# dhansmair/flamingo-mini

Measured on AMD Instinct MI355X. Metric: images/sec (fwd+bwd) flamingo-mini bs=32, higher is better.
Workload: dtype bf16

## Files before the change

flamingo-mini_amd/csrc/ff_api.hip:

```cpp
#include <stdarg.h>
#include <stdio.h>
#include <math.h>
#include <stdlib.h>
#include "ff_common.h"
#include "ff_internal.h"

namespace ff {

static thread_local char g_err[512] = "";
void set_error(const char* fmt, ...) {
    va_list ap;
    va_start(ap, fmt);
    vsnprintf(g_err, sizeof(g_err), fmt, ap);
    va_end(ap);
}
#ifdef FF_DEBUG
int dbg_switch(const char* name, int dflt) {
    const char* e = getenv(name);
    return e ? atoi(e) : dflt;
}
#endif
int check_launch(const char* what) {
    hipError_t e = hipGetLastError();
    if (e != hipSuccess) {
// ... 50 lines not shown
};
static void rs_take_layer_saved(const RsDims& s, Arena& a, RsLayerSaved& L) {
    const size_t rows_q = s.Mq, rows_kv = s.Mkv;
    L.mean_l = a.take<float>(rows_q * 4);
    L.rstd_l = a.take<float>(rows_q * 4);
    L.kv_in = a.take(rows_kv * s.D * s.es);
    L.Qs = a.take(rows_q * s.inner * s.es);
    L.K = a.take(rows_kv * s.inner * s.es);
    L.V = a.take(rows_kv * s.inner * s.es);
    L.lse = a.take<float>((size_t)s.Bn * s.H * s.q * 4);
    L.O = a.take(rows_q * s.inner * s.es);
    L.x_mid = a.take(rows_q * s.D * s.es);
    L.mean_f = a.take<float>(rows_q * 4);
    L.rstd_f = a.take<float>(rows_q * 4);
    L.xn_f = a.take(rows_q * s.D * s.es);
    L.Hpre = a.take(rows_q * s.ffi * s.es);
    L.Aact = a.take(rows_q * s.ffi * s.es);
}
static size_t rs_saved_layout(const RsDims& s, void* base, size_t cap, RsSaved& o) {
    Arena a(base, cap);
    const size_t rows_q = s.Mq;
    o.mean_m = a.take<float>((size_t)s.Mf * 4);
    o.rstd_m = a.take<float>((size_t)s.Mf * 4);
    for (int l = 0; l < s.depth; l++) {
        o.L[l].x_in = l == 0 ? nullptr : a.take(rows_q * s.D * s.es);
        rs_take_layer_saved(s, a, o.L[l]);
    }
    o.x_last = a.take(rows_q * s.D * s.es);
    o.mean_o = a.take<float>(rows_q * 4);
    o.rstd_o = a.take<float>(rows_q * 4);
    return align_up(a.used);
}

static size_t rs_ws_bytes(const RsDims& s) {
    size_t w = 0;
    auto g = [&](int M, int N, int K, int nz) { w = std::max(w, gemm_workspace_bytes(s.dt, M, N, K, nz, 0)); };
    g(s.Mq, s.inner, s.D, 1); g(s.Mkv, s.inner, s.D, 2); g(s.Mq, s.D, s.inner, 1); g(s.Mq, s.ffi, s.D, 1); g(s.Mq, s.D, s.ffi, 1);
    for (int nz = 1; nz <= 4; nz++) {
        g(s.D, s.ffi, s.Mq, nz); g(s.ffi, s.D, s.Mq, nz); g(s.D, s.inner, s.Mq, nz); g(s.inner, s.D, s.Mq, nz); g(s.inner, s.D, s.Mkv, nz);
    }
    g(s.Mkv, s.D, s.inner, 1);
    w = std::max(w, layernorm_bwd_workspace(s.Mf, s.D));
    w = std::max(w, layernorm_bwd_workspace(s.Mq, s.D));
    w = std::max(w, rows_reduce_workspace(s.Mq, s.D, s.q, 1));
    w = std::max(w, rows_reduce_workspace(s.Mf, s.D, s.F, s.v));
    return align_up(w) + align_up(s.attn_ws);
}
struct RsChain {
    void *ws, *dxn, *dO, *dkv, *dln;
    size_t ws_bytes, gws;
    float* attn_ws;
};
struct RsLayerGrads {
    void *dx_mid, *dH, *dQs, *dK, *dV;
};
static void rs_take_ws(const RsDims& s, Arena& a, RsChain& c) {
    c.ws_bytes = rs_ws_bytes(s);
    c.ws = a.take(c.ws_bytes);
    c.gws = c.ws_bytes - align_up(s.attn_ws);
    c.attn_ws = c.ws ? (float*)((char*)c.ws + c.gws) : nullptr;
}
static void rs_take_chain(const RsDims& s, Arena& a, RsChain& c) {
    c.dxn = a.take((size_t)s.Mq * s.D * s.es);
    c.dO = a.take((size_t)s.Mq * s.inner * s.es);
    c.dkv = a.take((size_t)s.Mkv * s.D * s.es);
    c.dln = a.take((size_t)s.Mq * s.D * s.es);
}
static void rs_take_layer_grads(const RsDims& s, Arena& a, RsLayerGrads& g) {
    g.dx_mid = a.take((size_t)s.Mq * s.D * s.es);
    g.dH = a.take((size_t)s.Mq * s.ffi * s.es);
    g.dQs = a.take((size_t)s.Mq * s.inner * s.es);
    g.dK = a.take((size_t)s.Mkv * s.inner * s.es);
    g.dV = a.take((size_t)s.Mkv * s.inner * s.es);
}
static void rs_take_ln_partials(const RsDims& s, Arena& a, bool deferrable, float** lnp) {
    for (int i = 0; i < 3; i++) lnp[i] = deferrable ? a.take<float>(layernorm_bwd_partial_bytes(i == 2 ? s.Mf : s.Mq, s.D)) : nullptr;
}

struct RsScratch {
    RsChain c;
    void *dx0, *dxf;
    void* dx_out[kMaxDepth];
    RsLayerGrads L[kMaxDepth];
    float* lnp[3 * kMaxDepth + 1];
};
static size_t rs_scratch_layout(const RsDims& s, void* base, size_t cap, bool bwd, RsScratch& o) {
    Arena a(base, cap);
    rs_take_ws(s, a, o.c);
    if (bwd) {
        o.dx0 = a.take((size_t)s.Mq * s.D * s.es);
        rs_take_chain(s, a, o.c);
        o.dxf = a.take((size_t)s.Mf * s.D * s.es);
        for (int l = 0; l < s.depth; l++) {
            o.dx_out[l] = a.take((size_t)s.Mq * s.D * s.es);
            rs_take_layer_grads(s, a, o.L[l]);
        }
        static const int defer_ln = dbg_switch("FF_DEFER_LN", 1);
        const bool lnd = defer_ln != 0 && layernorm_bwd_deferrable(s.dt, s.D);
        for (int l = 0; l < s.depth; l++) rs_take_ln_partials(s, a, lnd, o.lnp + 3 * l);
        o.lnp[3 * s.depth] = lnd ? a.take<float>(layernorm_bwd_partial_bytes(s.Mq, s.D)) : nullptr;
    }
    return align_up(a.used);
}

static int rs_check(const ff_resampler_desc* d) {
    FF_CHECK(d, FF_ERR_SHAPE, "resampler: null descriptor");
    FF_CHECK(d->dtype == FF_DTYPE_F32 || d->dtype == FF_DTYPE_BF16, FF_ERR_UNSUPPORTED, "resampler: dtype %d", d->dtype);
    FF_CHECK(d->batch > 0 && d->n_frames > 0 && d->n_tokens > 0 && d->dim > 0 && d->depth > 0 && d->depth <= kMaxDepth && d->heads > 0 &&
                 d->dim_head > 0 && d->num_latents > 0 && d->ff_mult > 0,
             FF_ERR_SHAPE, "resampler: bad dimensions");
    FF_CHECK(d->n_frames <= d->num_time_embeds, FF_ERR_SHAPE, "resampler: %d frames > num_time_embeds %d (perceiver_resampler.py:166)",
             d->n_frames, d->num_time_embeds);
    FF_CHECK(d->act >= FF_ACT_GELU && d->act <= FF_ACT_RELU, FF_ERR_SHAPE, "resampler: act %d", d->act);
    return FF_OK;
}

static ff_attn_desc rs_attn_desc(const RsDims& s) {
    ff_attn_desc a = {};
    a.dtype = s.dt; a.batch = s.Bn; a.heads = s.H; a.dim_head = s.dh; a.n_q = s.q; a.n_kv = s.R; a.mode = FF_ATTN_DENSE;
    const ff_strides sq = {(long long)s.q * s.inner, s.inner, s.dh}, sk = {(long long)s.R * s.inner, s.inner, s.dh};
    a.q = sq; a.o = sq; a.dq = sq; a.dout = sq;
    a.k = sk; a.v = sk; a.dk = sk; a.dv = sk;
    return a;
}

static int rs_media_stats(const RsDims& s, const void* x_f, const void* tpe, float* mean_m, float* rstd_m, hipStream_t st) {
    return layernorm_fwd(s.ln_media(s.pD), x_f, tpe, nullptr, nullptr, nullptr, mean_m, rstd_m, st);
}

static int rs_layer_forward(const RsDims& s, const void* const* p, const void* x_f, const void* tpe, float* mean_m, float* rstd_m, const void* x_in,
                            RowMap x_map, void* x_out, const RsLayerSaved& L, void* ws, size_t ws_bytes, hipStream_t st) {
    const RowMap pD = s.pD, pI = s.pI, pF = s.pF;
    void* kv_lat_base = s.kv_latent_rows(L.kv_in);
    {
        LnArgs a = s.ln_media(s.kv_media);
        a.stats_given = 1;
        FF_TRY(layernorm_fwd(a, x_f, tpe, p[0], p[1], L.kv_in, mean_m, rstd_m, st));
    }
    FF_TRY(layernorm_fwd(ln_args(s.dt, s.Mq, s.D, x_map, s.kv_lat, pD), x_in, nullptr, p[2], p[3], kv_lat_base, L.mean_l, L.rstd_l, st));
    FF_TRY(Gemm(s.dt, s.Mq, s.inner, s.D).a(0, s.kv_lat).b(0, pD).c(pI).scale(s.scale).problem(kv_lat_base, p[4], L.Qs).run(ws, ws_bytes, st));
    FF_TRY(Gemm(s.dt, s.Mkv, s.inner, s.D).a(0, pD).b(0, pD).c(pI).problem(L.kv_in, p[5], L.K).problem(L.kv_in, p[6], L.V).run(ws, ws_bytes, st));
    FF_TRY(attention_fwd(rs_attn_desc(s), L.Qs, L.K, L.V, nullptr, L.O, L.lse, st));
    FF_TRY(Gemm(s.dt, s.Mq, s.D, s.inner).a(0, pI).b(0, pI).c(pD).res_map(x_map).problem(L.O, p[7], L.x_mid, nullptr, nullptr, x_in).run(ws, ws_bytes, st));
    FF_TRY(layernorm_fwd(s.ln_latents(), L.x_mid, nullptr, p[8], p[9], L.xn_f, L.mean_f, L.rstd_f, st));
    FF_TRY(Gemm(s.dt, s.Mq, s.ffi, s.D).a(0, pD).b(0, pD).c(pF).act(s.act).problem(L.xn_f, p[10], L.Aact, L.Hpre).run(ws, ws_bytes, st));
    return Gemm(s.dt, s.Mq, s.D, s.ffi).a(0, pF).b(0, pF).c(pD).problem(L.Aact, p[11], x_out, nullptr, nullptr, L.x_mid).run(ws, ws_bytes, st);
}

static int rs_final_norm(const RsDims& s, const void* x_last, const void* gamma, const void* beta, void* out, float* mean, float* rstd, hipStream_t st) {
    return layernorm_fwd(s.ln_latents(), x_last, nullptr, gamma, beta, out, mean, rstd, st);
}

static int rs_ln_bwd(const RsChain& W, float* partial, LnPending* pending, const LnArgs& a, const void* dy, const void* x, const void* add,
                     const void* gamma, const float* mean, const float* rstd, void* dx, const void* dx_res, void* dg, void* db, hipStream_t st) {
    if (partial)
        return layernorm_bwd(a, dy, x, add, gamma, mean, rstd, dx, dx_res, dg, db, partial, layernorm_bwd_partial_bytes(a.rows, a.cols), st, nullptr, pending);
    return layernorm_bwd(a, dy, x, add, gamma, mean, rstd, dx, dx_res, dg, db, W.ws, W.gws, st);
}

static int rs_layer_backward(const RsDims& s, const void* const* p, void* const* g, const void* x_f, const void* tpe, const float* mean_m,
                             const float* rstd_m, const void* x_in, RowMap x_map, const RsLayerSaved& L, const void* dx_out, void* dx_in,
                             void* dx_f, const void* dx_f_res, const RsChain& W, const RsLayerGrads& T, float* const* lnp, LnPending* ln_sets,
                             hipStream_t st) {
    const RowMap pD = s.pD, pI = s.pI, pF = s.pF;
    FF_TRY(Gemm(s.dt, s.Mq, s.ffi, s.D).a(0, pD).b(1, pF).c(pF).act_bwd(s.act).problem(dx_out, p[11], T.dH, nullptr, L.Hpre).run(W.ws, W.gws, st));
    FF_TRY(Gemm(s.dt, s.Mq, s.D, s.ffi).a(0, pF).b(1, pD).c(pD).problem(T.dH, p[10], W.dxn).run(W.ws, W.gws, st));
    FF_TRY(rs_ln_bwd(W, lnp[0], &ln_sets[0], s.ln_latents(), W.dxn, L.x_mid, nullptr, p[8], L.mean_f, L.rstd_f, T.dx_mid, dx_out, g[8], g[9], st));
    FF_TRY(Gemm(s.dt, s.Mq, s.inner, s.D).a(0, pD).b(1, pI).c(pI).problem(T.dx_mid, p[7], W.dO).run(W.ws, W.gws, st));
    FF_TRY(attention_bwd(rs_attn_desc(s), L.Qs, L.K, L.V, nullptr, L.O, W.dO, L.lse, T.dQs, T.dK, T.dV, W.attn_ws, s.attn_ws, st));
    FF_TRY(Gemm(s.dt, s.Mkv, s.D, s.inner).a(0, pI).b(1, pD).c(pD).problem(T.dK, p[5], W.dkv).run(W.ws, W.gws, st));
    FF_TRY(Gemm(s.dt, s.Mkv, s.D, s.inner).a(0, pI).b(1, pD).c(pD).problem(T.dV, p[6], W.dkv, nullptr, nullptr, W.dkv).run(W.ws, W.gws, st));
    FF_TRY(Gemm(s.dt, s.Mq, s.D, s.inner).a(0, pI).b(1, pD).c(pD).res_map(s.kv_lat).scale(s.scale)
               .problem(T.dQs, p[4], W.dln, nullptr, nullptr, s.kv_latent_rows(W.dkv)).run(W.ws, W.gws, st));
    FF_TRY(rs_ln_bwd(W, lnp[1], &ln_sets[1], ln_args(s.dt, s.Mq, s.D, x_map, pD, pD), W.dln, x_in, nullptr, p[2], L.mean_l, L.rstd_l, dx_in, T.dx_mid, g[2],
                     g[3], st));
    return rs_ln_bwd(W, lnp[2], &ln_sets[2], s.ln_media(s.kv_media), W.dkv, x_f, tpe, p[0], mean_m, rstd_m, dx_f, dx_f_res, g[0], g[1], st);
}

static int rs_input_grads(const RsDims& s, const void* dx0, const void* dxf, void* d_latents, void* d_tpe, void* ws, size_t ws_bytes, hipStream_t st) {
    FF_TRY(rows_reduce(s.dt, s.Mq, s.D, s.pD, s.q, 1, dx0, d_latents, ws, ws_bytes, st));
    if (s.nte > s.T) FF_TRY(zero_bytes((char*)d_tpe + (size_t)s.T * s.D * s.es, (size_t)(s.nte - s.T) * s.D * s.es, st));
    return rows_reduce(s.dt, s.Mf, s.D, s.pD, s.F, s.v, dxf, d_tpe, ws, ws_bytes, st);
}

static int resampler_fwd(const ff_resampler_desc* d, const void* x_f, const void* const* P, void* out, void* saved, size_t saved_bytes,
                         void* scratch, size_t scratch_bytes, hipStream_t st) {
    FF_TRY(rs_check(d));
    FF_CHECK(x_f && P && out && saved && scratch, FF_ERR_SHAPE, "resampler_fwd: null argument");
    const RsDims s(*d);
    RsSaved S;
    RsScratch W;
    FF_CHECK(rs_saved_layout(s, saved, saved_bytes, S) <= saved_bytes, FF_ERR_WORKSPACE, "resampler_fwd: saved buffer too small");
    FF_CHECK(rs_scratch_layout(s, scratch, scratch_bytes, false, W) <= scratch_bytes, FF_ERR_WORKSPACE, "resampler_fwd: scratch too small");
    const void *latents = P[0], *tpe = P[1];
    FF_TRY(rs_media_stats(s, x_f, tpe, S.mean_m, S.rstd_m, st));
    for (int l = 0; l < s.depth; l++) {
        const void* const* p = P + FF_RESAMPLER_GLOBAL_PARAMS + FF_RESAMPLER_LAYER_PARAMS * l;
        void* x_next = l + 1 < s.depth ? S.L[l + 1].x_in : S.x_last;
        FF_TRY(rs_layer_forward(s, p, x_f, tpe, S.mean_m, S.rstd_m, l == 0 ? latents : S.L[l].x_in, l == 0 ? s.lat_bcast : s.pD, x_next, S.L[l], W.c.ws,
                                W.c.ws_bytes, st));
    }
    return rs_final_norm(s, S.x_last, P[2], P[3], out, S.mean_o, S.rstd_o, st);
}

static int resampler_bwd(const ff_resampler_desc* d, const void* x_f, const void* const* P, const void* dout, const void* saved,
                         size_t saved_bytes, void* const* G, void* dx_f, void* scratch, size_t scratch_bytes, hipStream_t st) {
    FF_TRY(rs_check(d));
    FF_CHECK(x_f && P && dout && saved && G && scratch, FF_ERR_SHAPE, "resampler_bwd: null argument");
    const RsDims s(*d);
    RsSaved S;
    RsScratch W;
    FF_CHECK(rs_saved_layout(s, (void*)saved, saved_bytes, S) <= saved_bytes, FF_ERR_WORKSPACE, "resampler_bwd: saved buffer too small");
    FF_CHECK(rs_scratch_layout(s, scratch, scratch_bytes, true, W) <= scratch_bytes, FF_ERR_WORKSPACE, "resampler_bwd: scratch too small");
    const RowMap pD = s.pD, pI = s.pI, pF = s.pF;
    const void *latents = P[0], *tpe = P[1];
    void* dxf = dx_f ? dx_f : W.dxf;
    void* const ws = W.c.ws;
    const size_t gws = W.c.gws;

    LnPending ln_sets[3 * kMaxDepth + 1];
    FF_TRY(rs_ln_bwd(W.c, W.lnp[3 * s.depth], &ln_sets[3 * s.depth], s.ln_latents(), dout, S.x_last, nullptr, P[2], S.mean_o, S.rstd_o,
                     W.dx_out[s.depth - 1], nullptr, G[2], G[3], st));
    for (int l = s.depth - 1; l >= 0; l--) {
        const void* const* p = P + FF_RESAMPLER_GLOBAL_PARAMS + FF_RESAMPLER_LAYER_PARAMS * l;
        void* const* g = G + FF_RESAMPLER_GLOBAL_PARAMS + FF_RESAMPLER_LAYER_PARAMS * l;
        void* dx_below = l == 0 ? W.dx0 : W.dx_out[l - 1];
        FF_TRY(rs_layer_backward(s, p, g, x_f, tpe, S.mean_m, S.rstd_m, l == 0 ? latents : S.L[l].x_in, l == 0 ? s.lat_bcast : pD, S.L[l], W.dx_out[l],
                                 dx_below, dxf, l == s.depth - 1 ? nullptr : dxf, W.c, W.L[l], W.lnp + 3 * l, ln_sets + 3 * l, st));
    }
    FF_TRY(layernorm_bwd_finish(s.dt, ln_sets, 3 * s.depth + 1, st));
    constexpr int kRsGroup = 4;
    for (int l0 = 0; l0 < s.depth; l0 += kRsGroup) {
        const int l1 = std::min(s.depth, l0 + kRsGroup);
        Gemm g3(s.dt, s.D, s.ffi, s.Mq), g1(s.dt, s.ffi, s.D, s.Mq), go(s.dt, s.D, s.inner, s.Mq), gq(s.dt, s.inner, s.D, s.Mq);
        g3.a(1, pD).b(1, pF).c(pF);
        g1.a(1, pF).b(1, pD).c(pD);
        go.a(1, pD).b(1, pI).c(pI);
        gq.a(1, pI).b(1, s.kv_lat).c(pD).scale(s.scale);
        for (int l = l0; l < l1; l++) {
            void* const* g = G + FF_RESAMPLER_GLOBAL_PARAMS + FF_RESAMPLER_LAYER_PARAMS * l;
            const RsLayerSaved& L = S.L[l];
            const RsLayerGrads& T = W.L[l];
            g3.problem(W.dx_out[l], L.Aact, g[11]);
            g1.problem(T.dH, L.xn_f, g[10]);
            go.problem(T.dx_mid, L.O, g[7]);
            gq.problem(T.dQs, s.kv_latent_rows(L.kv_in), g[4]);
        }
        FF_TRY(g3.run(ws, gws, st));
        FF_TRY(g1.run(ws, gws, st));
        FF_TRY(go.run(ws, gws, st));
        FF_TRY(gq.run(ws, gws, st));
    }
    {
        Gemm gkv(s.dt, s.inner, s.D, s.Mkv);
        gkv.a(1, pI).b(1, pD).c(pD);
        for (int l = 0; l < s.depth; l++) {
            void* const* g = G + FF_RESAMPLER_GLOBAL_PARAMS + FF_RESAMPLER_LAYER_PARAMS * l;
            gkv.problem(W.L[l].dK, S.L[l].kv_in, g[5]);
            gkv.problem(W.L[l].dV, S.L[l].kv_in, g[6]);
            if (gkv.P.nz == kRsGroup || l == s.depth - 1) {
                FF_TRY(gkv.run(ws, gws, st));
// ... 673 lines not shown
```

flamingo-mini_amd/csrc/ff_internal.h:

```cpp
#pragma once
#include <algorithm>
#include "ff_common.h"

namespace ff {

constexpr int kGemmMaxZ = 12;
constexpr int kKvProjGroup = 4;
struct GemmProblem {
    const void* A;
    const void* B;
    void* C;
    void* aux_out;
    const void* aux_in;
    const void* residual;
    const void* gate;
};
struct GemmParams {
    int M, N, K;
    int a_layout, b_layout;
    RowMap a_map, b_map, c_map, r_map;
    float scale;
    int act, act_bwd;
    int split_k, k_per_split;
    int tile;
// ... 19 lines not shown
        P.a_map = plain_rows(K); P.b_map = plain_rows(K); P.c_map = plain_rows(N); P.r_map = P.c_map;
    }
    Gemm& a(int layout, RowMap m) { P.a_layout = layout; P.a_map = m; return *this; }
    Gemm& b(int layout, RowMap m) { P.b_layout = layout; P.b_map = m; return *this; }
    Gemm& c(RowMap m) { P.c_map = m; P.r_map = m; return *this; }
    Gemm& res_map(RowMap m) { P.r_map = m; return *this; }
    Gemm& scale(float s) { P.scale = s; return *this; }
    Gemm& act(int a) { P.act = a; return *this; }
    Gemm& act_bwd(int a) { P.act_bwd = a; return *this; }
    Gemm& problem(const void* A, const void* B, void* C, void* aux_out = nullptr, const void* aux_in = nullptr,
                  const void* residual = nullptr, const void* gate = nullptr) {
        P.p[P.nz++] = GemmProblem{A, B, C, aux_out, aux_in, residual, gate};
        return *this;
    }
    size_t workspace() const { return gemm_workspace_bytes(dtype, P.M, P.N, P.K, std::max(P.nz, 1), P.split_k); }
    int run(void* ws, size_t ws_bytes, hipStream_t st, int* leave_partial = nullptr) const { return gemm_launch(P, dtype, ws, ws_bytes, st, leave_partial); }
};

int profile_begin(int dtype, int tile, int a_layout, int b_layout, int M, int N, int K, int nz, int split_k, hipStream_t st);
void profile_end(int i, hipStream_t st);

struct LnArgs {
    int dtype;
    int rows, cols;
    RowMap x_map, y_map, dx_map;
    int add_rows_per_seg, add_div;
    float eps;
    int stats_given;
    int dy_splits = 0;
    long long dy_slab = 0;
};
int layernorm_fwd(const LnArgs& a, const void* x, const void* add, const void* gamma, const void* beta, void* y,
                  float* mean, float* rstd, hipStream_t st);
size_t layernorm_bwd_workspace(int rows, int cols);
struct LnDots {
    const void* a = nullptr; const void* alpha_a = nullptr; void* out_a = nullptr;
    const void* b = nullptr; const void* alpha_b = nullptr; void* out_b = nullptr;
};
struct LnPending {
    const float* partial = nullptr;
    int nblk = 0, cols = 0;
    void *dgamma = nullptr, *dbeta = nullptr;
    const void* alpha_a = nullptr; void* out_a = nullptr;
    const void* alpha_b = nullptr; void* out_b = nullptr;
};
constexpr int kLnFinishMax = 8;
bool layernorm_bwd_deferrable(int dtype, int cols);
size_t layernorm_bwd_partial_bytes(int rows, int cols);
int layernorm_bwd_partial_blocks(int rows);
int layernorm_bwd(const LnArgs& a, const void* dy, const void* x, const void* add, const void* gamma, const float* mean,
                  const float* rstd, void* dx, const void* dx_residual, void* dgamma, void* dbeta, void* ws,
                  size_t ws_bytes, hipStream_t st, const LnDots* dots = nullptr, LnPending* pending = nullptr);
int layernorm_bwd_finish(int dtype, const LnPending* sets, int n, hipStream_t st);
size_t rows_reduce_workspace(int rows, int cols, int rows_per_batch, int rows_per_group);
int zero_bytes(void* p, size_t bytes, hipStream_t st);
int rows_reduce(int dtype, int rows, int cols, RowMap x_map, int rows_per_batch, int rows_per_group, const void* x,
                void* out, void* ws, size_t ws_bytes, hipStream_t st);
size_t gate_grad_workspace(int rows, int cols);
int gate_grad(int dtype, int rows, int cols, const void* a, const void* b, const void* alpha, void* dalpha, void* ws,
              size_t ws_bytes, hipStream_t st);
int text_time(int batch, int n_tokens, const void* ml, int elem_bytes, int* out, hipStream_t st);

size_t attention_bwd_workspace(const ff_attn_desc& d);
int attention_fwd(const ff_attn_desc& d, const void* Q, const void* K, const void* V, const int* tt, void* O, float* lse,
                  hipStream_t st);
int attention_bwd(const ff_attn_desc& d, const void* Q, const void* K, const void* V, const int* tt, const void* O,
// ... 59 lines not shown
```

flamingo-mini_amd/csrc/ff_rowwise.hip:

```cpp
#include "ff_common.h"
#include "ff_internal.h"

namespace ff {

#ifdef FF_XA_TIMELINE
__device__ unsigned long long g_ln_timeline[4096 * 8];
#define FF_LTL(i) do { if (threadIdx.x == 0 && blockIdx.x < 4096) g_ln_timeline[blockIdx.x * 8 + (i)] = __builtin_amdgcn_s_memrealtime(); } while (0)
#else
#define FF_LTL(i) do { } while (0)
#endif

template <typename T, int VEC> FF_DEV void ld(const T* p, float (&o)[VEC]) {
    if constexpr (VEC == 1) o[0] = to_f32(p[0]);
    else Vec<T>::load(p, o);
}
template <typename T, int VEC> FF_DEV void st(T* p, const float (&o)[VEC]) {
    if constexpr (VEC == 1) p[0] = from_f32<T>(o[0]);
    else Vec<T>::store(p, o);
}

template <typename T, int VEC>
__global__ __launch_bounds__(256) void ln_fwd_kernel(const LnArgs a_in, const T* __restrict__ x, const T* __restrict__ add,
                                                     const T* __restrict__ gamma, const T* __restrict__ beta, T* __restrict__ y,
                                                     float* __restrict__ mean, float* __restrict__ rstd) {
// ... 84 lines not shown
            float v[VEC];
            ld<T, VEC>(xr + c * VEC, v);
            if (ar) {
                float t[VEC];
                ld<T, VEC>(ar + c * VEC, t);
#pragma unroll
                for (int i = 0; i < VEC; i++) v[i] += t[i];
            }
#pragma unroll
            for (int i = 0; i < VEC; i++) q += (v[i] - mu) * (v[i] - mu);
        }
        rs = rsqrtf(wave_sum(q) / (float)a.cols + a.eps);
        if (lane == 0 && mean) {
            mean[row] = mu;
            rstd[row] = rs;
        }
    }
    if (!y) return;
    T* yr = y + a.y_map.off(row);
    for (int c = lane; c < nchunk; c += 64) {
        float v[VEC], g[VEC], b[VEC];
        ld<T, VEC>(xr + c * VEC, v);
        if (ar) {
            float t[VEC];
            ld<T, VEC>(ar + c * VEC, t);
#pragma unroll
            for (int i = 0; i < VEC; i++) v[i] += t[i];
        }
        ld<T, VEC>(gamma + c * VEC, g);
        ld<T, VEC>(beta + c * VEC, b);
#pragma unroll
        for (int i = 0; i < VEC; i++) v[i] = (v[i] - mu) * rs * g[i] + b[i];
        st<T, VEC>(yr + c * VEC, v);
    }
}

template <typename T, int VEC>
__global__ __launch_bounds__(256) void ln_bwd_dx_kernel(const LnArgs a_in, const T* __restrict__ dy, const T* __restrict__ x,
                                                        const T* __restrict__ add, const T* __restrict__ gamma,
                                                        const float* __restrict__ mean, const float* __restrict__ rstd, T* dx,
                                                        const T* dx_res) {
    const LnArgs a = fetch_args(a_in);
    pin_args(dy, x, add, gamma, mean, rstd, dx, dx_res);
    const int lane = threadIdx.x & 63;
    const int row = blockIdx.x * 4 + (threadIdx.x >> 6);
    if (row >= a.rows) return;
    const T* xr = x + a.x_map.off(row);
    const T* dyr = dy + a.y_map.off(row);
    const T* ar = nullptr;
    if (add) ar = add + (long long)((row % a.add_rows_per_seg) / a.add_div) * a.cols;
    const float mu = mean[row], rs = rstd[row];
    const int nchunk = a.cols / VEC;
    float s1 = 0.f, s2 = 0.f;
    for (int c = lane; c < nchunk; c += 64) {
        float v[VEC], d[VEC], g[VEC];
        ld<T, VEC>(xr + c * VEC, v);
        if (ar) {
            float t[VEC];
            ld<T, VEC>(ar + c * VEC, t);
#pragma unroll
            for (int i = 0; i < VEC; i++) v[i] += t[i];
        }
        ld<T, VEC>(dyr + c * VEC, d);
        ld<T, VEC>(gamma + c * VEC, g);
#pragma unroll
        for (int i = 0; i < VEC; i++) {
// ... 171 lines not shown
    }
    FF_LTL(2);
    {
        float* mine = sacc + (size_t)w * 2 * a.cols;
#pragma unroll
        for (int i = 0; i < NCH; i++) {
            const int c = lane + 64 * i;
            if (c < nchunk) {
#pragma unroll
                for (int e = 0; e < VEC; e += 4) {
                    *(f32x4*)(mine + c * VEC + e) = f32x4{accg[i][e], accg[i][e + 1], accg[i][e + 2], accg[i][e + 3]};
                    *(f32x4*)(mine + a.cols + c * VEC + e) = f32x4{accb[i][e], accb[i][e + 1], accb[i][e + 2], accb[i][e + 3]};
                }
            }
        }
    }
    __syncthreads();
    FF_LTL(3);
    const long long P = 2LL * a.cols + 2;
    float* out = partial + (long long)blockIdx.x * P;
    for (int i = threadIdx.x * 4; i < 2 * a.cols; i += 256 * 4) {
        const f32x4 s0 = *(const f32x4*)(sacc + i), s1 = *(const f32x4*)(sacc + 2 * a.cols + i);
        const f32x4 s2 = *(const f32x4*)(sacc + 4 * a.cols + i), s3 = *(const f32x4*)(sacc + 6 * a.cols + i);
        float* o = out + i;
        o[0] = (s0[0] + s1[0]) + (s2[0] + s3[0]); o[1] = (s0[1] + s1[1]) + (s2[1] + s3[1]);
        o[2] = (s0[2] + s1[2]) + (s2[2] + s3[2]); o[3] = (s0[3] + s1[3]) + (s2[3] + s3[3]);
    }
    da = block_sum<4>(da, red);
    db = block_sum<4>(db, red);
    if (threadIdx.x == 0) { out[2 * a.cols] = da; out[2 * a.cols + 1] = db; }
    FF_LTL(4);
}

template <typename T>
FF_DEV void ln_final_body(int nblk, int cols, const float* __restrict__ partial, T* dgamma, T* dbeta, const T* alpha_a, T* out_a, const T* alpha_b,
                          T* out_b) {
    __shared__ float red[16][17];
    const int P = 2 * cols + 2;
    const int tx = threadIdx.x & 15, ty = threadIdx.x >> 4;
    const int idx = blockIdx.x * 16 + tx;
    float v[8] = {0.f, 0.f, 0.f, 0.f, 0.f, 0.f, 0.f, 0.f};
    if (idx < P) {
        int b = ty;
        for (; b + 7 * 16 < nblk; b += 8 * 16) {
#pragma unroll
            for (int u = 0; u < 8; u++) v[u] += partial[(long long)(b + 16 * u) * P + idx];
        }
        for (; b < nblk; b += 16) v[0] += partial[(long long)b * P + idx];
    }
    red[ty][tx] = ((v[0] + v[1]) + (v[2] + v[3])) + ((v[4] + v[5]) + (v[6] + v[7]));
    __syncthreads();
    if (ty == 0 && idx < P) {
        float s = 0.f;
#pragma unroll
        for (int u = 0; u < 16; u++) s += red[u][tx];
        const float v = s;
        if (idx < cols) { if (dgamma) dgamma[idx] = from_f32<T>(v); }
        else if (idx < 2 * cols) { if (dbeta) dbeta[idx - cols] = from_f32<T>(v); }
        else if (idx == 2 * cols) {
            if (out_a) { const float t = tanhf(to_f32(alpha_a[0])); out_a[0] = from_f32<T>(v * (1.f - t * t)); }
        } else if (out_b) { const float t = tanhf(to_f32(alpha_b[0])); out_b[0] = from_f32<T>(v * (1.f - t * t)); }
    }
}
template <typename T>
__global__ __launch_bounds__(256) void ln_bwd_final_kernel(int nblk, int cols, const float* __restrict__ partial, T* dgamma, T* dbeta,
                                                           const T* alpha_a, T* out_a, const T* alpha_b, T* out_b) {
// ... 150 lines not shown
static bool vec_ok(int dtype, int cols, std::initializer_list<RowMap> maps, std::initializer_list<const void*> ptrs) {
    const int n = dtype == FF_DTYPE_BF16 ? 8 : 4;
    if (cols % n) return false;
    for (const RowMap& m : maps)
        if (m.ld % n || (m.rows_per_seg > 0 && m.seg_stride % n)) return false;
    for (const void* p : ptrs)
        if (p && (uintptr_t)p % 16) return false;
    return true;
}

#define FF_DISPATCH_T_VEC(dtype, vec, ...)                 \
    do {                                                    \
        if ((dtype) == FF_DTYPE_BF16) {                     \
            typedef bf16 T;                                 \
            if (vec) { constexpr int VEC = 8; __VA_ARGS__; }       \
            else { constexpr int VEC = 1; __VA_ARGS__; }           \
        } else {                                            \
            typedef float T;                                \
            if (vec) { constexpr int VEC = 4; __VA_ARGS__; }       \
            else { constexpr int VEC = 1; __VA_ARGS__; }           \
        }                                                   \
    } while (0)

int layernorm_fwd(const LnArgs& a, const void* x, const void* add, const void* gamma, const void* beta, void* y, float* mean,
                  float* rstd, hipStream_t st_) {
    FF_CHECK(a.rows > 0 && a.cols > 0 && x, FF_ERR_SHAPE, "layernorm_fwd: bad shape rows=%d cols=%d", a.rows, a.cols);
    FF_CHECK(!a.stats_given || (mean && rstd), FF_ERR_SHAPE, "layernorm_fwd: stats_given without statistics");
    FF_CHECK(!y || (gamma && beta), FF_ERR_SHAPE, "layernorm_fwd: gamma/beta missing");
    FF_CHECK(!add || (a.add_rows_per_seg > 0 && a.add_div > 0), FF_ERR_SHAPE, "layernorm_fwd: addend needs add_rows_per_seg/add_div");
    const bool v = vec_ok(a.dtype, a.cols, {a.x_map, a.y_map}, {x, add, gamma, beta, y});
    const int grid = cdiv(a.rows, 4);
    FF_DISPATCH_T_VEC(a.dtype, v, ln_fwd_kernel<T, VEC><<<dim3(grid), dim3(256), 0, st_>>>(a, (const T*)x, (const T*)add, (const T*)gamma, (const T*)beta, (T*)y, mean, rstd));
    return check_launch("ln_fwd");
}

static void split_plan(int n_rows_in_group, int col_blocks, int ngroups, int& rows_per_split, int& nsplit) {
    int target = std::max(1, 512 / std::max(1, col_blocks * ngroups));
    nsplit = std::max(1, std::min(std::min(target, 32), cdiv(n_rows_in_group, 32)));
    rows_per_split = cdiv(n_rows_in_group, nsplit);
    nsplit = cdiv(n_rows_in_group, rows_per_split);
}

static size_t col_reduce_ws(int n_rows_in_group, int cols, int ngroups, int nslots) {
    int rps, ns;
    split_plan(n_rows_in_group, 1, ngroups, rps, ns);
    return (size_t)ns * ngroups * nslots * cols * sizeof(float);
}


static int ln_fused_blocks(int rows, int& rows_per_block) {
    rows_per_block = std::max(4, (cdiv(rows, 256) + 3) / 4 * 4);
    return cdiv(rows, rows_per_block);
}
static bool ln_fused_ok(int dtype, int cols, bool vec) {
    if (!vec) return false;
    const int n = dtype == FF_DTYPE_BF16 ? 8 : 4;
    return cdiv(cols / n, 64) <= 8 && (size_t)8 * cols * sizeof(float) <= 150 * 1024;
}
size_t layernorm_bwd_workspace(int rows, int cols) {
    int rpb;
    const size_t fused = (size_t)ln_fused_blocks(rows, rpb) * (2 * (size_t)cols + 2) * sizeof(float);
    return std::max(fused, col_reduce_ws(rows, cols, 1, 2));
}

bool layernorm_bwd_deferrable(int dtype, int cols) { return cols % (dtype == FF_DTYPE_BF16 ? 8 : 4) == 0 && ln_fused_ok(dtype, cols, true); }
int layernorm_bwd_partial_blocks(int rows) {
// ... 61 lines not shown
        if (a.dtype == FF_DTYPE_BF16) return launch_ln_fused<bf16, 8>(a, dy, x, add, gamma, mean, rstd, dx, dx_residual, dots, dgamma, dbeta, (float*)ws, st_, pending);
        return launch_ln_fused<float, 4>(a, dy, x, add, gamma, mean, rstd, dx, dx_residual, dots, dgamma, dbeta, (float*)ws, st_, pending);
    }
    if (dots.a) FF_TRY(gate_grad(a.dtype, a.rows, a.cols, dx_residual, dots.a, dots.alpha_a, dots.out_a, ws, ws_bytes, st_));
    if (dx) {
        const int grid = cdiv(a.rows, 4);
        FF_DISPATCH_T_VEC(a.dtype, v, ln_bwd_dx_kernel<T, VEC><<<dim3(grid), dim3(256), 0, st_>>>(a, (const T*)dy, (const T*)x, (const T*)add, (const T*)gamma, mean, rstd, (T*)dx, (const T*)dx_residual));
        FF_TRY(check_launch("ln_bwd_dx"));
    }
    if (dgamma || dbeta) {
        FF_CHECK(dgamma && dbeta, FF_ERR_SHAPE, "layernorm_bwd: dgamma and dbeta come together");
        const int vecn = v ? (a.dtype == FF_DTYPE_BF16 ? 8 : 4) : 1;
        ColReduceArgs c = {};
        c.rows = a.rows; c.cols = a.cols; c.x_map = a.x_map; c.y_map = a.y_map;
        c.rows_per_batch = a.rows; c.rows_per_group = a.rows; c.n_batch = 1; c.ngroups = 1;
        c.add_rows_per_seg = a.add_rows_per_seg; c.add_div = a.add_div;
        const int col_blocks = cdiv(a.cols, 64 * vecn);
        split_plan(a.rows, col_blocks, 1, c.rows_per_split, c.nsplit);
        const size_t need = (size_t)c.nsplit * 2 * a.cols * sizeof(float);
        FF_CHECK(ws && ws_bytes >= need, FF_ERR_WORKSPACE, "layernorm_bwd workspace: need %zu have %zu", need, ws_bytes);
        FF_DISPATCH_T_VEC(a.dtype, v, col_reduce_kernel<T, VEC, 1><<<dim3(col_blocks, 1, c.nsplit), dim3(256), 0, st_>>>(c, (const T*)x, (const T*)dy, (const T*)add, mean, rstd, (float*)ws));
        FF_TRY(check_launch("ln_bwd_param_partial"));
        const int grid = std::min(cdiv(2LL * a.cols, 256), 1024);
        if (a.dtype == FF_DTYPE_BF16)
            hipLaunchKernelGGL(col_reduce_final_kernel<bf16>, dim3(grid), dim3(256), 0, st_, c.nsplit, 1, 2, a.cols, (const float*)ws, (bf16*)dgamma, (bf16*)dbeta);
        else
            hipLaunchKernelGGL(col_reduce_final_kernel<float>, dim3(grid), dim3(256), 0, st_, c.nsplit, 1, 2, a.cols, (const float*)ws, (float*)dgamma, (float*)dbeta);
        FF_TRY(check_launch("ln_bwd_param_final"));
    }
    if (dots.b) FF_TRY(gate_grad(a.dtype, a.rows, a.cols, dx, dots.b, dots.alpha_b, dots.out_b, ws, ws_bytes, st_));
    return FF_OK;
}

int layernorm_bwd_finish(int dtype, const LnPending* sets, int n, hipStream_t st_) {
    for (int i0 = 0; i0 < n; i0 += kLnFinishMax) {
        LnFinishTable t = {};
        int cnt = 0, pmax = 0;
        for (int i = i0; i < n && i < i0 + kLnFinishMax; i++)
            if (sets[i].partial) {
                t.s[cnt++] = sets[i];
                pmax = std::max(pmax, 2 * sets[i].cols + 2);
            }
        if (!cnt) continue;
        const dim3 grid(cdiv(pmax, 16), cnt);
        if (dtype == FF_DTYPE_BF16) ln_bwd_final_multi_kernel<bf16><<<grid, dim3(256), 0, st_>>>(t);
        else ln_bwd_final_multi_kernel<float><<<grid, dim3(256), 0, st_>>>(t);
        FF_TRY(check_launch("ln_bwd_final_multi"));
    }
    return FF_OK;
}

size_t rows_reduce_workspace(int rows, int cols, int rows_per_batch, int rows_per_group) {
    if (rows_per_batch <= 0 || rows_per_group <= 0) return 0;
    const int ngroups = cdiv(rows_per_batch, rows_per_group);
    const int n_batch = cdiv(rows, rows_per_batch);
    return col_reduce_ws(n_batch * rows_per_group, cols, ngroups, 1);
}

int rows_reduce(int dtype, int rows, int cols, RowMap x_map, int rows_per_batch, int rows_per_group, const void* x, void* out,
                void* ws, size_t ws_bytes, hipStream_t st_) {
    FF_CHECK(rows > 0 && cols > 0 && rows_per_batch > 0 && rows_per_group > 0 && x && out, FF_ERR_SHAPE, "rows_reduce: bad arguments");
    FF_CHECK(rows % rows_per_batch == 0 && rows_per_batch % rows_per_group == 0, FF_ERR_SHAPE,
             "rows_reduce: rows=%d rows_per_batch=%d rows_per_group=%d do not nest", rows, rows_per_batch, rows_per_group);
    const bool v = vec_ok(dtype, cols, {x_map}, {x, out});
    const int vecn = v ? (dtype == FF_DTYPE_BF16 ? 8 : 4) : 1;
    ColReduceArgs c = {};
// ... 102 lines not shown
```

Before: 785.1.

## Batch per-layer media layernorms across resampler layers into multi-output kernels

Every resampler layer layer-normalises the same media features with its own gamma and beta. Those per-layer forward layernorms now run as one kernel that reads x once and writes every layer's output. In backward, the media layernorm gradients of up to six layers are held in separate dkv buffers and processed together by one multi-set kernel that accumulates dx and the per-layer gamma/beta partials. This cuts repeated reads of the large media tensor and the number of launches, at the cost of extra scratch memory, more register pressure and a changed accumulation order in dx.

New measurement: 787.1 (median of 6 runs). About the same (+0.3%).

```diff
diff --git a/flamingo-mini_amd/csrc/ff_api.hip b/flamingo-mini_amd/csrc/ff_api.hip
--- a/flamingo-mini_amd/csrc/ff_api.hip
+++ b/flamingo-mini_amd/csrc/ff_api.hip
@@ -106,6 +106,12 @@
     return align_up(a.used);
 }
 
+constexpr size_t kRsMediaScratch = (size_t)256 << 20;
+static int rs_media_group(const RsDims& s) {
+    const size_t per_layer = align_up((size_t)s.Mkv * s.D * s.es);
+    return (int)std::max<size_t>(1, std::min<size_t>(std::min(s.depth, kLnMultiMax), kRsMediaScratch / per_layer));
+}
+
 static size_t rs_ws_bytes(const RsDims& s) {
     size_t w = 0;
     auto g = [&](int M, int N, int K, int nz) { w = std::max(w, gemm_workspace_bytes(s.dt, M, N, K, nz, 0)); };
@@ -157,6 +163,7 @@
     void* dx_out[kMaxDepth];
     RsLayerGrads L[kMaxDepth];
     float* lnp[3 * kMaxDepth + 1];
+    void* dkv[kLnMultiMax];
 };
 static size_t rs_scratch_layout(const RsDims& s, void* base, size_t cap, bool bwd, RsScratch& o) {
     Arena a(base, cap);
@@ -173,6 +180,9 @@
         const bool lnd = defer_ln != 0 && layernorm_bwd_deferrable(s.dt, s.D);
         for (int l = 0; l < s.depth; l++) rs_take_ln_partials(s, a, lnd, o.lnp + 3 * l);
         o.lnp[3 * s.depth] = lnd ? a.take<float>(layernorm_bwd_partial_bytes(s.Mq, s.D)) : nullptr;
+        static const int media_multi = dbg_switch("FF_RS_MEDIA_MULTI", 1);
+        const int mg = lnd && media_multi ? rs_media_group(s) : 0;
+        for (int i = 0; i < kLnMultiMax; i++) o.dkv[i] = i >= mg ? nullptr : i == 0 ? o.c.dkv : a.take((size_t)s.Mkv * s.D * s.es);
     }
     return align_up(a.used);
 }
@@ -202,11 +212,24 @@
     return layernorm_fwd(s.ln_media(s.pD), x_f, tpe, nullptr, nullptr, nullptr, mean_m, rstd_m, st);
 }
 
+static int rs_media_forward(const RsDims& s, const void* const* P, int l0, int l1, const void* x_f, const void* tpe, const float* mean_m,
+                            const float* rstd_m, const RsLayerSaved* L, hipStream_t st) {
+    LnArgs a = s.ln_media(s.kv_media);
+    a.stats_given = 1;
+    LnMultiFwd t = {};
+    for (int l = l0; l < l1; l++) {
+        const void* const* p = P + FF_RESAMPLER_GLOBAL_PARAMS + FF_RESAMPLER_LAYER_PARAMS * l;
+        t.gamma[l - l0] = p[0]; t.beta[l - l0] = p[1]; t.y[l - l0] = L[l].kv_in;
+    }
+    return layernorm_fwd_multi(a, x_f, tpe, mean_m, rstd_m, l1 - l0, t, st);
+}
+
 static int rs_layer_forward(const RsDims& s, const void* const* p, const void* x_f, const void* tpe, float* mean_m, float* rstd_m, const void* x_in,
-                            RowMap x_map, void* x_out, const RsLayerSaved& L, void* ws, size_t ws_bytes, hipStream_t st) {
+                            RowMap x_map, void* x_out, const RsLayerSaved& L, void* ws, size_t ws_bytes, hipStream_t st,
+                            bool media_done = false) {
     const RowMap pD = s.pD, pI = s.pI, pF = s.pF;
     void* kv_lat_base = s.kv_latent_rows(L.kv_in);
-    {
+    if (!media_done) {
         LnArgs a = s.ln_media(s.kv_media);
         a.stats_given = 1;
         FF_TRY(layernorm_fwd(a, x_f, tpe, p[0], p[1], L.kv_in, mean_m, rstd_m, st));
@@ -235,7 +258,7 @@
 static int rs_layer_backward(const RsDims& s, const void* const* p, void* const* g, const void* x_f, const void* tpe, const float* mean_m,
                              const float* rstd_m, const void* x_in, RowMap x_map, const RsLayerSaved& L, const void* dx_out, void* dx_in,
                              void* dx_f, const void* dx_f_res, const RsChain& W, const RsLayerGrads& T, float* const* lnp, LnPending* ln_sets,
-                             hipStream_t st) {
+                             hipStream_t st, bool media_later = false) {
     const RowMap pD = s.pD, pI = s.pI, pF = s.pF;
     FF_TRY(Gemm(s.dt, s.Mq, s.ffi, s.D).a(0, pD).b(1, pF).c(pF).act_bwd(s.act).problem(dx_out, p[11], T.dH, nullptr, L.Hpre).run(W.ws, W.gws, st));
     FF_TRY(Gemm(s.dt, s.Mq, s.D, s.ffi).a(0, pF).b(1, pD).c(pD).problem(T.dH, p[10], W.dxn).run(W.ws, W.gws, st));
@@ -248,7 +271,29 @@
                .problem(T.dQs, p[4], W.dln, nullptr, nullptr, s.kv_latent_rows(W.dkv)).run(W.ws, W.gws, st));
     FF_TRY(rs_ln_bwd(W, lnp[1], &ln_sets[1], ln_args(s.dt, s.Mq, s.D, x_map, pD, pD), W.dln, x_in, nullptr, p[2], L.mean_l, L.rstd_l, dx_in, T.dx_mid, g[2],
                      g[3], st));
+    if (media_later) return FF_OK;
     return rs_ln_bwd(W, lnp[2], &ln_sets[2], s.ln_media(s.kv_media), W.dkv, x_f, tpe, p[0], mean_m, rstd_m, dx_f, dx_f_res, g[0], g[1], st);
+}
+
+static void rs_media_bwd_table(const RsDims& s, const void* const* P, void* const* G, void* const* dkv, float* const* lnp, int l0, int l1,
+                               LnMultiBwd& t) {
+    t = LnMultiBwd{};
+    for (int i = 0; i < l1 - l0; i++) {
+        const int l = l1 - 1 - i;
+        const void* const* p = P + FF_RESAMPLER_GLOBAL_PARAMS + FF_RESAMPLER_LAYER_PARAMS * l;
+        void* const* g = G + FF_RESAMPLER_GLOBAL_PARAMS + FF_RESAMPLER_LAYER_PARAMS * l;
+        t.dy[i] = dkv[i]; t.gamma[i] = p[0]; t.partial[i] = lnp[3 * l + 2]; t.dgamma[i] = g[0]; t.dbeta[i] = g[1];
+    }
+}
+static int rs_media_backward(const RsDims& s, const void* const* P, void* const* G, int l0, int l1, bool first, const void* x_f, const void* tpe,
+                             const float* mean_m, const float* rstd_m, void* dxf, void* const* dkv, float* const* lnp, LnPending* ln_sets,
+                             hipStream_t st) {
+    LnMultiBwd t;
+    LnPending pend[kLnMultiMax];
+    rs_media_bwd_table(s, P, G, dkv, lnp, l0, l1, t);
+    FF_TRY(layernorm_bwd_multi(s.ln_media(s.kv_media), x_f, tpe, mean_m, rstd_m, dxf, first ? nullptr : dxf, l1 - l0, t, pend, st));
+    for (int i = 0; i < l1 - l0; i++) ln_sets[3 * (l1 - 1 - i) + 2] = pend[i];
+    return FF_OK;
 }
 
 static int rs_input_grads(const RsDims& s, const void* dx0, const void* dxf, void* d_latents, void* d_tpe, void* ws, size_t ws_bytes, hipStream_t st) {
@@ -268,11 +313,13 @@
     FF_CHECK(rs_scratch_layout(s, scratch, scratch_bytes, false, W) <= scratch_bytes, FF_ERR_WORKSPACE, "resampler_fwd: scratch too small");
     const void *latents = P[0], *tpe = P[1];
     FF_TRY(rs_media_stats(s, x_f, tpe, S.mean_m, S.rstd_m, st));
+    for (int l0 = 0; l0 < s.depth; l0 += kLnMultiMax)
+        FF_TRY(rs_media_forward(s, P, l0, std::min(s.depth, l0 + kLnMultiMax), x_f, tpe, S.mean_m, S.rstd_m, S.L, st));
     for (int l = 0; l < s.depth; l++) {
         const void* const* p = P + FF_RESAMPLER_GLOBAL_PARAMS + FF_RESAMPLER_LAYER_PARAMS * l;
         void* x_next = l + 1 < s.depth ? S.L[l + 1].x_in : S.x_last;
         FF_TRY(rs_layer_forward(s, p, x_f, tpe, S.mean_m, S.rstd_m, l == 0 ? latents : S.L[l].x_in, l == 0 ? s.lat_bcast : s.pD, x_next, S.L[l], W.c.ws,
-                                W.c.ws_bytes, st));
+                                W.c.ws_bytes, st, true));
     }
     return rs_final_norm(s, S.x_last, P[2], P[3], out, S.mean_o, S.rstd_o, st);
 }
@@ -293,14 +340,26 @@
     const size_t gws = W.c.gws;
 
     LnPending ln_sets[3 * kMaxDepth + 1];
+    const int mg = rs_media_group(s);
+    bool media_multi = W.dkv[0] != nullptr;
+    for (int l1 = s.depth; l1 > 0 && media_multi; l1 -= mg) {
+        LnMultiBwd t;
+        rs_media_bwd_table(s, P, G, W.dkv, W.lnp, std::max(0, l1 - mg), l1, t);
+        media_multi = layernorm_bwd_multi_ok(s.ln_media(s.kv_media), x_f, tpe, dxf, dxf, l1 - std::max(0, l1 - mg), t);
+    }
     FF_TRY(rs_ln_bwd(W.c, W.lnp[3 * s.depth], &ln_sets[3 * s.depth], s.ln_latents(), dout, S.x_last, nullptr, P[2], S.mean_o, S.rstd_o,
                      W.dx_out[s.depth - 1], nullptr, G[2], G[3], st));
     for (int l = s.depth - 1; l >= 0; l--) {
         const void* const* p = P + FF_RESAMPLER_GLOBAL_PARAMS + FF_RESAMPLER_LAYER_PARAMS * l;
         void* const* g = G + FF_RESAMPLER_GLOBAL_PARAMS + FF_RESAMPLER_LAYER_PARAMS * l;
         void* dx_below = l == 0 ? W.dx0 : W.dx_out[l - 1];
+        const int i = media_multi ? (s.depth - 1 - l) % mg : 0;
+        RsChain c = W.c;
+        c.dkv = media_multi ? W.dkv[i] : W.c.dkv;
         FF_TRY(rs_layer_backward(s, p, g, x_f, tpe, S.mean_m, S.rstd_m, l == 0 ? latents : S.L[l].x_in, l == 0 ? s.lat_bcast : pD, S.L[l], W.dx_out[l],
-                                 dx_below, dxf, l == s.depth - 1 ? nullptr : dxf, W.c, W.L[l], W.lnp + 3 * l, ln_sets + 3 * l, st));
+                                 dx_below, dxf, l == s.depth - 1 ? nullptr : dxf, c, W.L[l], W.lnp + 3 * l, ln_sets + 3 * l, st, media_multi));
+        if (media_multi && (i == mg - 1 || l == 0))
+            FF_TRY(rs_media_backward(s, P, G, l, l + i + 1, l + i + 1 == s.depth, x_f, tpe, S.mean_m, S.rstd_m, dxf, W.dkv, W.lnp, ln_sets, st));
     }
     FF_TRY(layernorm_bwd_finish(s.dt, ln_sets, 3 * s.depth + 1, st));
     constexpr int kRsGroup = 4;
diff --git a/flamingo-mini_amd/csrc/ff_internal.h b/flamingo-mini_amd/csrc/ff_internal.h
--- a/flamingo-mini_amd/csrc/ff_internal.h
+++ b/flamingo-mini_amd/csrc/ff_internal.h
@@ -75,6 +75,25 @@
 };
 int layernorm_fwd(const LnArgs& a, const void* x, const void* add, const void* gamma, const void* beta, void* y,
                   float* mean, float* rstd, hipStream_t st);
+constexpr int kLnMultiMax = 6;
+struct LnMultiFwd {
+    const void* gamma[kLnMultiMax];
+    const void* beta[kLnMultiMax];
+    void* y[kLnMultiMax];
+};
+int layernorm_fwd_multi(const LnArgs& a, const void* x, const void* add, const float* mean, const float* rstd, int n, const LnMultiFwd& t,
+                        hipStream_t st);
+struct LnPending;
+struct LnMultiBwd {
+    const void* dy[kLnMultiMax];
+    const void* gamma[kLnMultiMax];
+    float* partial[kLnMultiMax];
+    void* dgamma[kLnMultiMax];
+    void* dbeta[kLnMultiMax];
+};
+bool layernorm_bwd_multi_ok(const LnArgs& a, const void* x, const void* add, const void* dx, const void* dx_residual, int n, const LnMultiBwd& t);
+int layernorm_bwd_multi(const LnArgs& a, const void* x, const void* add, const float* mean, const float* rstd, void* dx, const void* dx_residual,
+                        int n, const LnMultiBwd& t, LnPending* pending, hipStream_t st);
 size_t layernorm_bwd_workspace(int rows, int cols);
 struct LnDots {
     const void* a = nullptr; const void* alpha_a = nullptr; void* out_a = nullptr;
diff --git a/flamingo-mini_amd/csrc/ff_rowwise.hip b/flamingo-mini_amd/csrc/ff_rowwise.hip
--- a/flamingo-mini_amd/csrc/ff_rowwise.hip
+++ b/flamingo-mini_amd/csrc/ff_rowwise.hip
@@ -140,6 +140,56 @@
 #pragma unroll
         for (int i = 0; i < VEC; i++) v[i] = (v[i] - mu) * rs * g[i] + b[i];
         st<T, VEC>(yr + c * VEC, v);
+    }
+}
+
+template <typename T, int VEC>
+__global__ __launch_bounds__(256) void ln_fwd_multi_kernel(const LnArgs a_in, const T* __restrict__ x, const T* __restrict__ add,
+                                                           const float* __restrict__ mean, const float* __restrict__ rstd, int n,
+                                                           const LnMultiFwd t) {
+    const LnArgs a = fetch_args(a_in);
+    pin_args(x, add, mean, rstd, n);
+    const int lane = threadIdx.x & 63;
+    const int row = blockIdx.x * 4 + (threadIdx.x >> 6);
+    if (row >= a.rows) return;
+    const T* xr = x + a.x_map.off(row);
+    const T* ar = nullptr;
+    if (add) ar = add + (long long)((row % a.add_rows_per_seg) / a.add_div) * a.cols;
+    const int nchunk = a.cols / VEC;
+    const float mu = mean[row], rs = rstd[row];
+    const long long yoff = a.y_map.off(row);
+    auto load_row = [&](int c, float (&v)[VEC]) {
+        ld<T, VEC>(xr + c * VEC, v);
+        if (ar) {
+            float s[VEC];
+            ld<T, VEC>(ar + c * VEC, s);
+#pragma unroll
+            for (int i = 0; i < VEC; i++) v[i] += s[i];
+        }
+    };
+    auto write = [&](int l, int c, const float (&v)[VEC]) {
+        float g[VEC], b[VEC], o[VEC];
+        ld<T, VEC>((const T*)t.gamma[l] + c * VEC, g);
+        ld<T, VEC>((const T*)t.beta[l] + c * VEC, b);
+#pragma unroll
+        for (int i = 0; i < VEC; i++) o[i] = (v[i] - mu) * rs * g[i] + b[i];
+        st<T, VEC>((T*)t.y[l] + yoff + c * VEC, o);
+    };
+    if (nchunk <= 4 * 64 && VEC > 1) {
+        float v[4][VEC];
+#pragma unroll
+        for (int u = 0; u < 4; u++)
+            if (lane + 64 * u < nchunk) load_row(lane + 64 * u, v[u]);
+        for (int l = 0; l < n; l++)
+#pragma unroll
+            for (int u = 0; u < 4; u++)
+                if (lane + 64 * u < nchunk) write(l, lane + 64 * u, v[u]);
+        return;
+    }
+    for (int c = lane; c < nchunk; c += 64) {
+        float v[VEC];
+        load_row(c, v);
+        for (int l = 0; l < n; l++) write(l, c, v);
     }
 }
 
@@ -377,6 +427,126 @@
     FF_LTL(4);
 }
 
+FF_DEV float add_unfused(float a, float b) {
+#pragma clang fp contract(off)
+    return a + b;
+}
+
+template <typename T, int VEC, int NCH, int NL>
+__global__ __launch_bounds__(256) void ln_bwd_multi_kernel(const LnArgs a_in, const T* __restrict__ x, const T* __restrict__ add,
+                                                           const float* __restrict__ mean, const float* __restrict__ rstd, T* dx, const T* dx_res,
+                                                           int n, const LnMultiBwd t, int rows_per_block) {
+    const LnArgs a = fetch_args(a_in);
+    pin_args(x, add, mean, rstd, dx, dx_res, n, rows_per_block);
+    extern __shared__ __attribute__((aligned(16))) float sacc[];
+    const int lane = threadIdx.x & 63, w = threadIdx.x >> 6;
+    const int nchunk = a.cols / VEC;
+    float accg[NL][NCH][VEC], accb[NL][NCH][VEC];
+#pragma unroll
+    for (int l = 0; l < NL; l++)
+#pragma unroll
+        for (int i = 0; i < NCH; i++)
+#pragma unroll
+            for (int e = 0; e < VEC; e++) accg[l][i][e] = accb[l][i][e] = 0.f;
+    const int row_end = min(a.rows, (int)(blockIdx.x + 1) * rows_per_block);
+    for (int row = blockIdx.x * rows_per_block + w; row < row_end; row += 4) {
+        const T* xr = x + a.x_map.off(row);
+        const T* ar = add ? add + (long long)((row % a.add_rows_per_seg) / a.add_div) * a.cols : nullptr;
+        const float mu = mean[row], rs = rstd[row];
+        const long long yoff = a.y_map.off(row), doff = a.dx_map.off(row);
+        float xh[NCH][VEC], o[NCH][VEC];
+#pragma unroll
+        for (int i = 0; i < NCH; i++) {
+            const int c = lane + 64 * i;
+            if (c < nchunk) {
+                float v[VEC];
+                ld<T, VEC>(xr + c * VEC, v);
+                if (ar) {
+                    float s[VEC];
+                    ld<T, VEC>(ar + c * VEC, s);
+#pragma unroll
+                    for (int e = 0; e < VEC; e++) v[e] += s[e];
+                }
+#pragma unroll
+                for (int e = 0; e < VEC; e++) { xh[i][e] = (v[e] - mu) * rs; o[i][e] = 0.f; }
+                if (dx_res) ld<T, VEC>(dx_res + doff + c * VEC, o[i]);
+            }
+        }
+        bool have = dx_res != nullptr;
+#pragma unroll
+        for (int l = 0; l < NL; l++) {
+            if (l < n) {
+                const T* dyr = (const T*)t.dy[l] + yoff;
+                const T* gamma = (const T*)t.gamma[l];
+                float d[NCH][VEC], g[NCH][VEC];
+                float s1 = 0.f, s2 = 0.f;
+#pragma unroll
+                for (int i = 0; i < NCH; i++) {
+                    const int c = lane + 64 * i;
+                    if (c < nchunk) {
+                        ld<T, VEC>(dyr + c * VEC, d[i]);
+                        ld<T, VEC>(gamma + c * VEC, g[i]);
+#pragma unroll
+                        for (int e = 0; e < VEC; e++) {
+                            const float dyh = d[i][e] * g[i][e];
+                            s1 += dyh;
+                            s2 += dyh * xh[i][e];
+                        }
+                    }
+                }
+                const float m1 = wave_sum(s1) / (float)a.cols, m2 = wave_sum(s2) / (float)a.cols;
+#pragma unroll
+                for (int i = 0; i < NCH; i++) {
+                    if (lane + 64 * i < nchunk) {
+#pragma unroll
+                        for (int e = 0; e < VEC; e++) {
+                            const float r = rs * (d[i][e] * g[i][e] - m1 - xh[i][e] * m2);
+                            o[i][e] = to_f32(from_f32<T>(have ? add_unfused(r, o[i][e]) : r));
+                            accg[l][i][e] += d[i][e] * xh[i][e];
+                            accb[l][i][e] += d[i][e];
+                        }
+                    }
+                }
+                have = true;
+            }
+        }
+#pragma unroll
+        for (int i = 0; i < NCH; i++) {
+            const int c = lane + 64 * i;
+            if (c < nchunk) st<T, VEC>(dx + doff + c * VEC, o[i]);
+        }
+    }
+    const long long P = 2LL * a.cols + 2;
+    float* mine = sacc + (size_t)w * 2 * a.cols;
+#pragma unroll
+    for (int l = 0; l < NL; l++) {
+        if (l < n) {
+#pragma unroll
+            for (int i = 0; i < NCH; i++) {
+                const int c = lane + 64 * i;
+                if (c < nchunk) {
+#pragma unroll
+                    for (int e = 0; e < VEC; e += 4) {
+                        *(f32x4*)(mine + c * VEC + e) = f32x4{accg[l][i][e], accg[l][i][e + 1], accg[l][i][e + 2], accg[l][i][e + 3]};
+                        *(f32x4*)(mine + a.cols + c * VEC + e) = f32x4{accb[l][i][e], accb[l][i][e + 1], accb[l][i][e + 2], accb[l][i][e + 3]};
+                    }
+                }
+            }
+            __syncthreads();
+            float* out = t.partial[l] + (long long)blockIdx.x * P;
+            for (int i = threadIdx.x * 4; i < 2 * a.cols; i += 256 * 4) {
+                const f32x4 s0 = *(const f32x4*)(sacc + i), s1 = *(const f32x4*)(sacc + 2 * a.cols + i);
+                const f32x4 s2 = *(const f32x4*)(sacc + 4 * a.cols + i), s3 = *(const f32x4*)(sacc + 6 * a.cols + i);
+                float* q = out + i;
+                q[0] = (s0[0] + s1[0]) + (s2[0] + s3[0]); q[1] = (s0[1] + s1[1]) + (s2[1] + s3[1]);
+                q[2] = (s0[2] + s1[2]) + (s2[2] + s3[2]); q[3] = (s0[3] + s1[3]) + (s2[3] + s3[3]);
+            }
+            if (threadIdx.x == 0) { out[2 * a.cols] = 0.f; out[2 * a.cols + 1] = 0.f; }
+            __syncthreads();
+        }
+    }
+}
+
 template <typename T>
 FF_DEV void ln_final_body(int nblk, int cols, const float* __restrict__ partial, T* dgamma, T* dbeta, const T* alpha_a, T* out_a, const T* alpha_b,
                           T* out_b) {
@@ -593,6 +763,21 @@
     const int grid = cdiv(a.rows, 4);
     FF_DISPATCH_T_VEC(a.dtype, v, ln_fwd_kernel<T, VEC><<<dim3(grid), dim3(256), 0, st_>>>(a, (const T*)x, (const T*)add, (const T*)gamma, (const T*)beta, (T*)y, mean, rstd));
     return check_launch("ln_fwd");
+}
+
+int layernorm_fwd_multi(const LnArgs& a, const void* x, const void* add, const float* mean, const float* rstd, int n, const LnMultiFwd& t,
+                        hipStream_t st_) {
+    FF_CHECK(a.rows > 0 && a.cols > 0 && x && mean && rstd && a.stats_given, FF_ERR_SHAPE, "layernorm_fwd_multi: bad arguments");
+    FF_CHECK(n >= 1 && n <= kLnMultiMax, FF_ERR_SHAPE, "layernorm_fwd_multi: %d outputs", n);
+    FF_CHECK(!add || (a.add_rows_per_seg > 0 && a.add_div > 0), FF_ERR_SHAPE, "layernorm_fwd_multi: addend needs add_rows_per_seg/add_div");
+    bool v = vec_ok(a.dtype, a.cols, {a.x_map, a.y_map}, {x, add});
+    for (int i = 0; i < n; i++) {
+        FF_CHECK(t.gamma[i] && t.beta[i] && t.y[i], FF_ERR_SHAPE, "layernorm_fwd_multi: null entry %d", i);
+        v = v && vec_ok(a.dtype, a.cols, {}, {t.gamma[i], t.beta[i], t.y[i]});
+    }
+    const int grid = cdiv(a.rows, 4);
+    FF_DISPATCH_T_VEC(a.dtype, v, ln_fwd_multi_kernel<T, VEC><<<dim3(grid), dim3(256), 0, st_>>>(a, (const T*)x, (const T*)add, mean, rstd, n, t));
+    return check_launch("ln_fwd_multi");
 }
 
 static void split_plan(int n_rows_in_group, int col_blocks, int ngroups, int& rows_per_split, int& nsplit) {
@@ -720,6 +905,61 @@
     return FF_OK;
 }
 
+bool layernorm_bwd_multi_ok(const LnArgs& a, const void* x, const void* add, const void* dx, const void* dx_residual, int n, const LnMultiBwd& t) {
+    bool v = a.dy_splits == 0 && vec_ok(a.dtype, a.cols, {a.x_map, a.y_map, a.dx_map}, {x, add, dx, dx_residual});
+    for (int i = 0; i < n && v; i++) v = t.partial[i] && vec_ok(a.dtype, a.cols, {}, {t.dy[i], t.gamma[i]});
+    return v && ln_fused_ok(a.dtype, a.cols, true);
+}
+
+template <typename T, int VEC, int NCH, int NL>
+static int launch_ln_multi(const LnArgs& a, const void* x, const void* add, const float* mean, const float* rstd, void* dx, const void* dx_res,
+                           int n, const LnMultiBwd& t, LnPending* pending, hipStream_t st_) {
+    int rpb;
+    const int nblk = ln_fused_blocks(a.rows, rpb);
+    const size_t lds = (size_t)8 * a.cols * sizeof(float);
+    if (lds > 48 * 1024) {
+        static bool attr[64] = {};
+        int dev = 0;
+        (void)hipGetDevice(&dev);
+        if (dev < 0 || dev >= 64 || !attr[dev]) {
+            hipFuncSetAttribute((const void*)ln_bwd_multi_kernel<T, VEC, NCH, NL>, hipFuncAttributeMaxDynamicSharedMemorySize, 150 * 1024);
+            if (dev >= 0 && dev < 64) attr[dev] = true;
+        }
+    }
+    for (int l0 = 0; l0 < n; l0 += NL) {
+        const int cnt = std::min(NL, n - l0);
+        LnMultiBwd u = {};
+        for (int i = 0; i < cnt; i++) {
+            u.dy[i] = t.dy[l0 + i]; u.gamma[i] = t.gamma[l0 + i]; u.partial[i] = t.partial[l0 + i];
+            LnPending& p = pending[l0 + i];
+            p = LnPending{};
+            p.partial = t.partial[l0 + i]; p.nblk = nblk; p.cols = a.cols; p.dgamma = t.dgamma[l0 + i]; p.dbeta = t.dbeta[l0 + i];
+        }
+        ln_bwd_multi_kernel<T, VEC, NCH, NL><<<dim3(nblk), dim3(256), lds, st_>>>(a, (const T*)x, (const T*)add, mean, rstd, (T*)dx,
+                                                                                  (const T*)(l0 == 0 ? dx_res : dx), cnt, u, rpb);
+        FF_TRY(check_launch("ln_bwd_multi"));
+    }
+    return FF_OK;
+}
+template <typename T, int VEC>
+static int dispatch_ln_multi(const LnArgs& a, const void* x, const void* add, const float* mean, const float* rstd, void* dx, const void* dx_res,
+                             int n, const LnMultiBwd& t, LnPending* pending, hipStream_t st_) {
+    const int nch = cdiv(a.cols / VEC, 64);
+    if (nch <= 2) return launch_ln_multi<T, VEC, 2, 6>(a, x, add, mean, rstd, dx, dx_res, n, t, pending, st_);
+    if (nch <= 4) return launch_ln_multi<T, VEC, 4, 3>(a, x, add, mean, rstd, dx, dx_res, n, t, pending, st_);
+    return launch_ln_multi<T, VEC, 8, 1>(a, x, add, mean, rstd, dx, dx_res, n, t, pending, st_);
+}
+
+int layernorm_bwd_multi(const LnArgs& a, const void* x, const void* add, const float* mean, const float* rstd, void* dx, const void* dx_residual,
+                        int n, const LnMultiBwd& t, LnPending* pending, hipStream_t st_) {
+    FF_CHECK(a.rows > 0 && a.cols > 0 && x && mean && rstd && dx && pending, FF_ERR_SHAPE, "layernorm_bwd_multi: null/shape");
+    FF_CHECK(n >= 1 && n <= kLnMultiMax, FF_ERR_SHAPE, "layernorm_bwd_multi: %d sets", n);
+    FF_CHECK(!add || (a.add_rows_per_seg > 0 && a.add_div > 0), FF_ERR_SHAPE, "layernorm_bwd_multi: addend needs add_rows_per_seg/add_div");
+    FF_CHECK(layernorm_bwd_multi_ok(a, x, add, dx, dx_residual, n, t), FF_ERR_UNSUPPORTED, "layernorm_bwd_multi: needs the one-pass kernel's shapes and alignment");
+    if (a.dtype == FF_DTYPE_BF16) return dispatch_ln_multi<bf16, 8>(a, x, add, mean, rstd, dx, dx_residual, n, t, pending, st_);
+    return dispatch_ln_multi<float, 4>(a, x, add, mean, rstd, dx, dx_residual, n, t, pending, st_);
+}
+
 int layernorm_bwd_finish(int dtype, const LnPending* sets, int n, hipStream_t st_) {
     for (int i0 = 0; i0 < n; i0 += kLnFinishMax) {
         LnFinishTable t = {};
```
